# peterdavidfagan/mujoco_robot_environments

Measured on AMD Instinct MI355X. Metric: env steps/sec (whole node), RearrangementEnv batch=4096 at 1/2/4/8 MI355X, higher is better.
Workload: dtype f32

## Files before the change

### mujoco_robot_environments_amd/csrc/mre_api.cpp

```cpp
#include <hip/hip_runtime.h>

#include <cmath>
#include <cstdio>
#include <cstdlib>
#include <cstring>
#include <string>
#include <algorithm>
#include <vector>

#include "mre_env.h"
#include "mre_launch.h"
#include "mre_model.h"

using namespace mre;

static thread_local std::string g_err;
int mre::fail(int code, const std::string& msg) {
  g_err = msg;
  return code;
}

extern "C" const char* mre_last_error(void) { return g_err.c_str(); }

static int create_buffers(mre_env* e, int num_envs, int device_id) {
// ... 20 lines not shown
  HIPCHK(hipStreamCreateWithFlags(&e->stream2, hipStreamNonBlocking));
  HIPCHK(hipEventCreateWithFlags(&e->ev_fork, hipEventDisableTiming));
  HIPCHK(hipEventCreateWithFlags(&e->ev_join, hipEventDisableTiming));
  HIPCHK(hipMalloc(&e->d_large, N)); HIPCHK(hipMalloc(&e->mask_r, N));
  HIPCHK(hipMalloc(&e->sv_qpos, N * NQP * 4)); HIPCHK(hipMalloc(&e->sv_qvel, N * NVP * 4));
  HIPCHK(hipMalloc(&e->sv_qacc_ws, N * NVP * 4)); HIPCHK(hipMalloc(&e->sv_ctrl, N * NU * 4));
  HIPCHK(hipMalloc(&e->sv_status, N * 4));
  HIPCHK(hipMalloc(&e->sv_converged, N));
  HIPCHK(hipHostMalloc((void**)&e->h_launch_info, mre_env::RING * N * 16, hipHostMallocMapped | hipHostMallocCoherent));
  HIPCHK(hipHostGetDevicePointer((void**)&e->d_launch_info, e->h_launch_info, 0));
  memset(e->h_launch_info, 0xFF, mre_env::RING * N * 16);
  HIPCHK(hipHostMalloc((void**)&e->h_info_last, N * 16, hipHostMallocDefault));
  memset(e->h_info_last, 0xFF, N * 16);
  HIPCHK(hipHostMalloc((void**)&e->h_large_stage, mre_env::NSTAGE * N, hipHostMallocMapped | hipHostMallocCoherent));
  HIPCHK(hipHostGetDevicePointer((void**)&e->d_large_stage, e->h_large_stage, 0));
  memset(e->h_large_stage, 0, mre_env::NSTAGE * N);
  HIPCHK(hipMalloc(&e->d_pending, N));
  HIPCHK(hipMemsetAsync(e->d_pending, 0, N, e->stream));
  HIPCHK(hipMemsetAsync(e->d_large, 0, N, e->stream));
  e->h_large.assign(N, 0); e->h_rerun.assign(N, 0);
  { int rc = sched_create(e); if (rc) return rc; }
  if (const char* fb = getenv("MRE_NO_FALLBACK")) e->fallback = atoi(fb) == 0;
  if (const char* ng = getenv("MRE_NARROW_GENERIC")) e->base_flags = atoi(ng) != 0 ? F_CLIP_ALWAYS : 0u;
  if (const char* ng = getenv("MRE_NEWTON_GENERIC")) e->base_flags |= atoi(ng) != 0 ? F_NW_ALL_TILES : 0u;
  if (const char* fl = getenv("MRE_FORCE_LARGE")) {
    if (atoi(fl) != 0) {
      e->h_large.assign(N, 1); e->n_large = num_envs;
      HIPCHK(hipMemsetAsync(e->d_large, 1, N, e->stream));
    }
  }
  HIPCHK(hipMemsetAsync(e->status, 0, N * 4, e->stream)); HIPCHK(hipMemsetAsync(e->stats, 0, N * 16, e->stream));
  HIPCHK(hipMemsetAsync(e->grip_closed, 0, N, e->stream)); HIPCHK(hipMemsetAsync(e->osc_target, 0, N * 64, e->stream));
  HIPCHK(hipMemsetAsync(e->sites, 0, N * 64, e->stream));
  std::vector<int> np(N, NPROP);
  std::vector<float> ps(N * NPROP * 3, 0.0155f);
  HIPCHK(hipMemcpy(e->nprops, np.data(), N * 4, hipMemcpyHostToDevice));
  HIPCHK(hipMemcpy(e->prop_size, ps.data(), ps.size() * 4, hipMemcpyHostToDevice));
  e->osc = OscConfig{350.f, 20.f, 500.f, 100.f, 200.f, 30.f, {0.f, -0.785f, 0.f, -2.356f, 0.f, 1.571f, 0.785f},
                     5e-3f, 68e-3f, 0};
  HIPCHK(hipMalloc(&e->d_osc, sizeof(OscConfig)));
  HIPCHK(hipMemcpy(e->d_osc, &e->osc, sizeof(OscConfig), hipMemcpyHostToDevice));
  HIPCHK(hipStreamSynchronize(e->stream));
  int rc = mre_reset(e, nullptr);
  if (rc != MRE_OK) return rc;
  return mre_sync(e);
}
// ... 993 lines not shown
```

### mujoco_robot_environments_amd/csrc/mre_collide.h

```cpp
#pragma once
#include "mre_math.h"

namespace mre {

constexpr int COLL_BUF = 48;
MRE_DEV float* cand_xyz(float* buf, int k) { return buf + 24 + 3 * k; }
MRE_DEV float& cand_dist(float* buf, int k) { return buf[3 * k + 2]; }

struct FaceCand { float x[4], y[4], z[4], d[4]; };
constexpr unsigned FACE_IN_REGS = 16u;
constexpr unsigned FACE_BRANCH = 32u;

MRE_DEV float sel3(const float* v, int i) {
  const float w0 = i == 0 ? 1.f : 0.f, w1 = i == 1 ? 1.f : 0.f, w2 = i == 2 ? 1.f : 0.f;
  return w0 * v[0] + w1 * v[1] + w2 * v[2];
}
MRE_DEV void row3(float* o, const float (*m)[3], int i) {
  const float w0 = i == 0 ? 1.f : 0.f, w1 = i == 1 ? 1.f : 0.f, w2 = i == 2 ? 1.f : 0.f;
  o[0] = w0 * m[0][0] + w1 * m[1][0] + w2 * m[2][0];
  o[1] = w0 * m[0][1] + w1 * m[1][1] + w2 * m[2][1];
  o[2] = w0 * m[0][2] + w1 * m[1][2] + w2 * m[2][2];
}

MRE_DEV int clip_poly(float* p, float* q, int n, float sx, float sy) {
// ... 307 lines not shown
    for (int k = 0; k < 3; k++) x[k] += t * a[k];
  }
  if (wn > 1e-4f) {
    for (int k = 0; k < 3; k++) x[k] -= r * w[k] / wn;
  } else {
    float o[3];
    for (int k = 0; k < 3; k++) o[k] = fminf(fmaxf(x[k], -sb[k]), sb[k]) - x[k];
    const float oa = o[0] * a[0] + o[1] * a[1] + o[2] * a[2];
    for (int k = 0; k < 3; k++) o[k] -= oa * a[k];
    const float on = sqrtf(o[0] * o[0] + o[1] * o[1] + o[2] * o[2]);
    const float sc = on > r ? r / on : 1.f;
    for (int k = 0; k < 3; k++) x[k] += sc * o[k];
  }
  for (int k = 0; k < 3; k++) x[k] -= 0.5f * best * bd[k];
  float* c0 = cand_xyz(buf, 0);
  for (int k = 0; k < 3; k++) {
    c0[k] = pb[k] + Rb[3 * k] * x[0] + Rb[3 * k + 1] * x[1] + Rb[3 * k + 2] * x[2];
    normal[k] = Rb[3 * k] * bd[0] + Rb[3 * k + 1] * bd[1] + Rb[3 * k + 2] * bd[2];
  }
  cand_dist(buf, 0) = best;
  return 1;
}

MRE_DEV void make_frame(float* f) {
  float y[3] = {0.f, 0.f, 0.f};
  if (f[1] < 0.5f && f[1] > -0.5f) y[1] = 1.f; else y[2] = 1.f;
  const float t = v3dot(f, y);
  v3addscl(y, f, -t);
  v3normalize(y);
  v3copy(f + 3, y);
  v3cross(f + 6, f, f + 3);
}

}
```

### mujoco_robot_environments_amd/csrc/mre_dev.h

```cpp
#pragma once
#include <stdint.h>

namespace mre {

constexpr int NB = 20;
constexpr int NRB = 16;
constexpr int GRIP_BODY0 = 8;
constexpr int NV = 39;
constexpr int NRV = 15;
constexpr int NQ = 43;
constexpr int NQP = 44;
constexpr int TRACE_W = 88;
constexpr int TRACE_QVEL = 48;
constexpr int NVP = 40;
constexpr int NU = 8;
constexpr int QFINE = 32;
constexpr int QFINE_ROW = 96;
constexpr int QFINE_CUBE_Q = 32;
constexpr int QFINE_CUBE_V = 60;
static_assert(QFINE_CUBE_Q + 7 * 4 == QFINE_CUBE_V && QFINE_CUBE_V + 6 * 4 <= QFINE_ROW, "qfine row layout");
constexpr int NPROP = 4;
constexpr int NG = 20;
constexpr int PROP_GEOM0 = 12;
constexpr int NPAIR = 128;
// ... 132 lines not shown
  PairRec pair_rec[NPAIR];
  float act_ctrlrange[NU][2];
  float home_qpos[7];
  float park_pos[NPROP][3];
  BodyRec body_rec[NB];
  DofRec dof_rec[NV];
  MEntryRec m_rec[NMR];
  RowRec row_rec[NROWREC];
  EqRec eq_rec[NEQ];
  SiteRec site_rec[NSITE];
  OptRec opt_rec;
};

struct OscConfig {
  float kp_pos, kd_pos, kp_ori, kd_ori, kp_null, kd_null;
  float null_q[7];
  float pos_thresh, ori_thresh;
  int pinv_always;
};

enum StepFlags : unsigned { F_NO_CONSTRAINTS = 1u, F_FREEZE_ROBOT = 2u, F_CONV_CONTINUE = 4u, F_CONV_OPEN = 8u,
                            F_OSC_EVAL = 16u, F_DETECT = 32u, F_SETTLE_EXIT = 64u, F_DETECT_ACTIVE = 128u,
                            F_CLIP_ALWAYS = 256u, F_NW_ALL_TILES = 512u };
enum CtrlMode : int { CTRL_HELD = 0, CTRL_SEQ = 1, CTRL_OSC = 2 };

struct StepArgs {
  const DevModel* M;
  int N;
  float* qpos;
  float* qvel;
  float* qacc_ws;
  float* qfine;
  float* ctrl;
  const float* ctrl_seq;
  int seq_stride;
  const int* nprops;
  const float* prop_size;
  int nsteps, control_steps, mode;
  unsigned flags;
  const OscConfig* osc;
  int osc_stride;
  const float* osc_target;
  const uint8_t* grip_closed;
  uint8_t* converged;
  float* sites;
  uint32_t* status;
// ... 114 lines not shown
```

### mujoco_robot_environments_amd/csrc/mre_kernels.hip

```cpp
#include <hip/hip_runtime.h>

#include "mre_dev.h"
#include "mre_math.h"
#include "mre_collide.h"

namespace mre {
using ModelP = MRE_MODEL_PTR(DevModel);
#if defined(MRE_PHASE_STAMPS) && MRE_PHASE_STAMPS >= 4
__shared__ unsigned long long dbg_acc[4];
#endif

struct OscSm {
  float J[6][7], M[7][7], MiJt[7][6], Li[6][6], Lam[6][6], V[6][6], Jbar[7][6];
  float ep[3], eo[3], F[6], LF[6], tn[7], Jbt[6], xd[6], w[6];
};

struct alignas(8) Blk {
  uint16_t row0;
  uint8_t type, nrows;
  uint8_t rslot;
  uint8_t pa, pb;
  uint8_t primary : 4;
  uint8_t bslot : 4;
};
// ... 1374 lines not shown
  for (int step = step_lo; step < step_hi; ++step) {
    MRE_STAMP(7);
    position_stage(M, s, l);
    MRE_STAMP(12);
    MRE_STAMP(13);
    gripper_local(M, s, l);
    if ((a.flags & F_NO_CONSTRAINTS) == 0) connect_rows_local(M, s, l);
    MRE_STAMP(14);
    crb_mass_matrix(M, s, l);
    MRE_SYNC();
#ifndef MRE_NEWTON
    factor_robot_regs(s.qM, s.qLD, s.qLDinv);
#endif
    MRE_STAMP(15);
    MRE_STAMP(0);

    velocity_stage(M, s, l);
    MRE_SYNC();
    finger_bias(M, s, l);
    MRE_STAMP(1);
    const bool constrained = (a.flags & F_NO_CONSTRAINTS) == 0;
    if (constrained) {

      collide(M, s, l, false, (a.flags & F_CLIP_ALWAYS) != 0);
      MRE_STAMP(2);
      assemble_constraints(M, s, l);
#ifdef MRE_NEWTON
      nw_build_lists(s, l, a.flags);
#else
      solve_robot_rows(s, l);
      assemble_blocks(M, s, l);
#endif
      MRE_STAMP(3);
      hw_ncon = max(hw_ncon, s.ncon); hw_nefc = max(hw_nefc, s.nefc);
      hw_nrrow = max(hw_nrrow, s.nrrow); hw_npp = max(hw_npp, s.npp);
    }

    if (a.mode == CTRL_SEQ && (step % a.control_steps) == 0) {
      const int tick = step / a.control_steps;
      if (l < NU) s.ctrl[l] = a.ctrl_seq[((size_t)tick * a.seq_stride + env) * NU + l];
      MRE_SYNC();
    }
    if (a.mode == CTRL_OSC && (step % a.control_steps) == 0) {
      if (step > 0 && osc_converged(M, s, oscp, s.osc_tgt)) arm_converged = true;
      osc_compute(M, s, osc, oscp, s.osc_tgt, l);
      if (l == 0) s.ctrl[NU - 1] = grip_cmd;
      MRE_SYNC();
// ... 69 lines not shown
    }
    if (settled) break;
  }
  MRE_STAMP(7);
  if (a.settle_steps != nullptr && l == 0) a.settle_steps[env] = settled ? steps_done : -steps_done;
  const bool hand_over = QUEUE && !Q_LARGE && s.overflow != 0;
  if (a.nstep != nullptr && l == 0 && !hand_over) {
    if (QUEUE) __hip_atomic_fetch_add(a.nstep + env, steps_done, __ATOMIC_RELAXED, __HIP_MEMORY_SCOPE_AGENT);
    else a.nstep[env] += steps_done;
  }
  if (a.nsteps == 0 && (a.flags & F_OSC_EVAL) != 0 && a.mode == CTRL_OSC) {
    position_stage(M, s, l);
    gripper_local(M, s, l);
    crb_mass_matrix(M, s, l);
    MRE_SYNC();
    velocity_stage(M, s, l);
    MRE_SYNC();
    osc_compute(M, s, osc, oscp, s.osc_tgt, l);
    if (l == 0) s.ctrl[NU - 1] = grip_cmd;
    MRE_SYNC();
  }
  if (a.nsteps == 0 && (a.flags & F_DETECT) != 0 && a.contacts != nullptr) {
    position_stage(M, s, l);
    collide(M, s, l, (a.flags & F_DETECT_ACTIVE) == 0, (a.flags & F_CLIP_ALWAYS) != 0);
    float* o = a.contacts + (size_t)env * (1 + 3 * CONTACT_EXPORT);
    const int n = s.ncon < CONTACT_EXPORT ? s.ncon : CONTACT_EXPORT;
    if (l == 0) o[0] = s.overflow ? -(float)s.ncon : (float)s.ncon;
    if (l < n) {
      const int pr = s.con_pair[l];
      o[1 + 3 * l] = (float)M->pair_g1[pr]; o[2 + 3 * l] = (float)M->pair_g2[pr]; o[3 + 3 * l] = s.con_dist[l];
      if (a.contacts_full != nullptr) {
        float* f = a.contacts_full + ((size_t)env * CONTACT_EXPORT + l) * 12;
        for (int k = 0; k < 3; k++) f[k] = s.con_pos[l][k];
        for (int k = 0; k < 9; k++) f[3 + k] = s.con_frame[l][k];
      }
    }
    MRE_SYNC();
    if (l == 0) s.overflow = 0;
  }
  const bool q_last = !QUEUE || (qtick + 1 == a.q_nticks && !hand_over);
  if (q_last && (a.mode == CTRL_OSC || a.sites != nullptr || a.geoms != nullptr)) kinematics_only(M, s, l);
  if (a.mode == CTRL_OSC && a.nsteps > 0 && !hand_over) {
    if (q_last && osc_converged(M, s, oscp, s.osc_tgt)) arm_converged = true;
    if (l == 0) {
      if (a.converged != nullptr) a.converged[env] = arm_converged ? 1 : 0;
      if (q_last && !arm_converged && a.status != nullptr && (a.flags & F_CONV_OPEN) == 0) {
        if (QUEUE) __hip_atomic_fetch_or(a.status + env, 1u, __ATOMIC_RELAXED, __HIP_MEMORY_SCOPE_AGENT);
// ... 485 lines not shown
```

### mujoco_robot_environments_amd/csrc/mre_solver.h

```cpp
#pragma once

namespace mre {

constexpr int HDR_NONE = 0xFF;
constexpr int BLK_NONE = 0x7F;
constexpr int SCHED_NONE = 0xFF;
constexpr int TAB_OFF = MAXBLK * 5;
constexpr int TAB_ZEROS = 48;
static_assert(TAB_BYTES == 8 * (TAB_OFF + 1) + 4 * TAB_ZEROS, "operand table size");

#ifndef MRE_NEWTON
MRE_DEV void build_schedule(ModelP M, Sm& s);
#endif
MRE_DEV constexpr int cube_pair_bit(int p, int q) {
  const int a = p < q ? p : q, b = p < q ? q : p;
  return a == 0 ? b - 1 : (a == 1 ? b + 1 : 5);
}

MRE_DEV float prop_invM(const Sm& s, int p, int k) {
  return 1.0f / ((k < 3) ? s.prop_mass[p] : s.prop_inertia[p][k - 3]);
}

MRE_DEV void geom_pose(ModelP M, const Sm& s, int g, float* p, float* R, float* size,
                       float* rbound) {
// ... 6 lines not shown
  const int pid = M->geom_propid[g];
  if (pid >= 0) {
    v3copy(size, s.prop_size[pid]);
    *rbound = v3norm(size);
  } else {
    v3copy(size, M->geom_size[g]);
    *rbound = M->geom_rbound[g];
  }
}

MRE_DEV void geom_center(ModelP M, const Sm& s, int g, float* p, float* rbound) {
  const int b = M->geom_body[g];
  float tmp[3];
  m3mulv(tmp, s.xmat[b], M->geom_pos[g]);
  v3add(p, s.xpos[b], tmp);
  const int pid = M->geom_propid[g];
  *rbound = pid >= 0 ? v3norm(s.prop_size[pid]) : M->geom_rbound[g];
}

MRE_PHASE_FN int collide_broad(ModelP M, Sm& s, int l, bool detect) {
  static_assert(offsetof(Sm, hdr) + sizeof(((Sm*)0)->hdr) - offsetof(Sm, JpA) >= sizeof(float) * 64 * COLL_BUF,
                "clip buffers do not fit");
  static_assert(NPAIR <= 256 && sizeof(((Sm*)0)->iscr) >= NPAIR, "survivor list: one byte per pair");
  MRE_DBG_T0();
  uint8_t* list = reinterpret_cast<uint8_t*>(s.iscr);
  const unsigned long long lt = (1ull << l) - 1ull;
  int nsurv = 0;
  for (int pass = 0; pass < NPAIR / 64; pass++) {
    const int pr = l + 64 * pass;
    const auto* R = &M->pair_rec[pr];
    const int g1 = R->g1, b1 = R->b1, b2 = R->b2, pid1 = R->pid1, pid2 = R->pid2, type1 = R->type1;
    const float lp1[3] = {R->pos1[0], R->pos1[1], R->pos1[2]}, lp2[3] = {R->pos2[0], R->pos2[1], R->pos2[2]};
    const float mrb1 = R->rb1, mrb2 = R->rb2, margin = R->margin, gap = R->gap;
    const float lq1[4] = {R->quat1[0], R->quat1[1], R->quat1[2], R->quat1[3]};
    bool live = false;
    if (g1 >= 0 && (pid1 < 0 || pid1 < s.nprops) && (pid2 < 0 || pid2 < s.nprops)) {
      const float inc = detect ? margin : margin - gap;
      float p1[3], p2[3], df[3], tmp[3];
      m3mulv(tmp, s.xmat[b1], lp1); v3add(p1, s.xpos[b1], tmp);
      m3mulv(tmp, s.xmat[b2], lp2); v3add(p2, s.xpos[b2], tmp);
      const float rb1 = pid1 >= 0 ? v3norm(s.prop_size[pid1]) : mrb1, rb2 = pid2 >= 0 ? v3norm(s.prop_size[pid2]) : mrb2;
      v3sub(df, p2, p1);
      if (type1 == 0) {
        float q[4], R1[9];
        qmul(q, s.xquat[b1], lq1);
        q2mat(R1, q);
        const float nn[3] = {R1[2], R1[5], R1[8]};
        live = v3dot(df, nn) - rb2 <= inc;
      } else {
        const float r = rb1 + rb2 + inc;
        live = v3dot(df, df) <= r * r;
      }
    }
    const unsigned long long m = __ballot(live);
    if (live) list[nsurv + __popcll(m & lt)] = (uint8_t)pr;
    nsurv += __popcll(m);
  }
  if (l == 0) s.ncon = 0;
  MRE_SYNC();
  MRE_DBG_STAMP(6, 0);
  return nsurv;
}
MRE_PHASE_FN int collide_narrow(ModelP M, Sm& s, int l, bool detect, bool clip_always, int c0, int nsurv, int base) {
  MRE_DBG_T0();
  float* buf = &s.JpA[0][0] + l * COLL_BUF;
  const uint8_t* list = reinterpret_cast<const uint8_t*>(s.iscr);
  const unsigned long long lt = (1ull << l) - 1ull;
  {
    const int pr = (c0 + l < nsurv) ? list[c0 + l] : -1;
    float normal[3] = {0.f, 0.f, 1.f};
    int n = 0;
    FaceCand rc;
    unsigned rm = 0u;
    if (pr >= 0) {
      const auto* R = &M->pair_rec[pr];
      const int b1 = R->b1, b2 = R->b2, pid1 = R->pid1, pid2 = R->pid2, type1 = R->type1;
      const float lp1[3] = {R->pos1[0], R->pos1[1], R->pos1[2]}, lp2[3] = {R->pos2[0], R->pos2[1], R->pos2[2]};
      const float lq1[4] = {R->quat1[0], R->quat1[1], R->quat1[2], R->quat1[3]};
      const float lq2[4] = {R->quat2[0], R->quat2[1], R->quat2[2], R->quat2[3]};
      const float ms1[3] = {R->size1[0], R->size1[1], R->size1[2]}, ms2[3] = {R->size2[0], R->size2[1], R->size2[2]};
      const float margin = R->margin, gap = R->gap;
      float p1[3], R1[9], s1[3], p2[3], R2[9], s2[3], tmp[3], q[4];
      m3mulv(tmp, s.xmat[b1], lp1); v3add(p1, s.xpos[b1], tmp);
      qmul(q, s.xquat[b1], lq1); q2mat(R1, q);
      m3mulv(tmp, s.xmat[b2], lp2); v3add(p2, s.xpos[b2], tmp);
      qmul(q, s.xquat[b2], lq2); q2mat(R2, q);
      if (pid1 >= 0) v3copy(s1, s.prop_size[pid1]); else v3copy(s1, ms1);
      if (pid2 >= 0) v3copy(s2, s.prop_size[pid2]); else v3copy(s2, ms2);
      const float inc = detect ? margin : margin - gap;
      MRE_DBG_STAMP(6, 1);
      if ((R->single >> 8) == 2) n = cyl_box(p1, R1, s1, p2, R2, s2[0], s2[2], inc, normal, buf);
      else if (type1 == 0) n = plane_box(p1, R1, p2, R2, s2, inc, normal, buf);
      else n = box_box(p1, R1, s1, p2, R2, s2, inc, normal, buf, clip_always, rc, rm);
      MRE_DBG_STAMP(6, 2);
      int m = 0;
      if (rm & FACE_IN_REGS) {
#pragma unroll
        for (int v = 0; v < 4; v++) {
          if (((rm >> v) & 1u) != 0u && rc.d[v] < inc) m++;
          else rm &= ~(1u << v);
        }
      } else {
        for (int c = 0; c < n; c++)
          if (cand_dist(buf, c) < inc) {
            if (m != c) {
              for (int k = 0; k < 3; k++) cand_xyz(buf, m)[k] = cand_xyz(buf, c)[k];
              cand_dist(buf, m) = cand_dist(buf, c);
            }
            m++;
          }
      }
      n = m;
    }
#if defined(MRE_PHASE_STAMPS) && MRE_PHASE_STAMPS == 8
    {
      const bool tbl = pr >= 0 && (M->pair_rec[pr].g1 == 1);
      const unsigned long long fb = __ballot((rm & FACE_BRANCH) != 0u), fr = __ballot((rm & FACE_IN_REGS) != 0u), tb = __ballot(tbl);
      if (l == 0) {
        dbg_acc[0] += (unsigned long long)__popcll(fb) << 4; dbg_acc[1] += (unsigned long long)__popcll(fr) << 4;
        dbg_acc[2] += (unsigned long long)__popcll(fb & tb) << 4; dbg_acc[3] += (unsigned long long)__popcll(fr & tb) << 4;
      }
    }
#endif
    const bool single = pr >= 0 && n > 1 && (M->pair_rec[pr].single & 0xFF) != 0;
    const int ncand = n;
    if (single) n = 1;
    int off = base, tot = base;
    for (int bit = 0; bit < 4; bit++) {
      const unsigned long long m = __ballot((n >> bit) & 1);
      off += __popcll(m & lt) << bit;
      tot += __popcll(m) << bit;
    }
    if (l == 0) {
      s.ncon = tot < NCON_MAX ? tot : NCON_MAX;
      if (tot > NCON_MAX) s.overflow = 1;
    }
    if (single) {
      const float incw = M->pair_rec[pr].margin - M->pair_rec[pr].gap;
      if (rm & FACE_IN_REGS) {
        float wsum = 0.f, px = 0.f, py = 0.f, pz = 0.f, dmin = 0.f, bx = 0.f, by = 0.f, bz = 0.f;
        bool first = true;
#pragma unroll
        for (int v = 0; v < 4; v++)
          if (((rm >> v) & 1u) != 0u) {
            const float dc = rc.d[v];
            if (first || dc < dmin) { dmin = dc; bx = rc.x[v]; by = rc.y[v]; bz = rc.z[v]; }
            first = false;
            const float w = incw - dc;
            if (w > 0.f) { wsum += w; px += w * rc.x[v]; py += w * rc.y[v]; pz += w * rc.z[v]; }
          }
        if (wsum > 0.f) { const float iw = 1.0f / wsum; px *= iw; py *= iw; pz *= iw; }
        else { px = bx; py = by; pz = bz; }
        rc.x[0] = px; rc.y[0] = py; rc.z[0] = pz; rc.d[0] = dmin;
        rm = FACE_IN_REGS | 1u;
      } else {
        float wsum = 0.f, px = 0.f, py = 0.f, pz = 0.f, dmin = cand_dist(buf, 0);
        int best = 0;
        for (int c = 0; c < ncand; c++) {
          const float dc = cand_dist(buf, c);
          if (dc < dmin) { dmin = dc; best = c; }
          const float w = incw - dc;
          if (w > 0.f) { wsum += w; px += w * cand_xyz(buf, c)[0]; py += w * cand_xyz(buf, c)[1]; pz += w * cand_xyz(buf, c)[2]; }
        }
        if (wsum > 0.f) { const float iw = 1.0f / wsum; px *= iw; py *= iw; pz *= iw; }
        else { px = cand_xyz(buf, best)[0]; py = cand_xyz(buf, best)[1]; pz = cand_xyz(buf, best)[2]; }
        cand_xyz(buf, 0)[0] = px; cand_xyz(buf, 0)[1] = py; cand_xyz(buf, 0)[2] = pz;
        cand_dist(buf, 0) = dmin;
      }
    }
    if (n > 0) {
      float f[9];
      v3copy(f, normal);
      make_frame(f);
      if (rm & FACE_IN_REGS) {
        int id = off;
#pragma unroll
        for (int v = 0; v < 4; v++)
          if (((rm >> v) & 1u) != 0u && id < NCON_MAX) {
            s.con_pos[id][0] = rc.x[v]; s.con_pos[id][1] = rc.y[v]; s.con_pos[id][2] = rc.z[v];
            for (int k = 0; k < 9; k++) s.con_frame[id][k] = f[k];
            s.con_dist[id] = rc.d[v];
            s.con_pair[id] = (uint8_t)pr;
            id++;
          }
      } else {
        for (int c = 0; c < n; c++) {
          const int id = off + c;
          if (id >= NCON_MAX) break;
          const float cx0 = cand_xyz(buf, c)[0], cx1 = cand_xyz(buf, c)[1], cx2 = cand_xyz(buf, c)[2];
          s.con_pos[id][0] = cx0; s.con_pos[id][1] = cx1; s.con_pos[id][2] = cx2;
          for (int k = 0; k < 9; k++) s.con_frame[id][k] = f[k];
          s.con_dist[id] = cand_dist(buf, c);
          s.con_pair[id] = (uint8_t)pr;
        }
      }
    }
    MRE_SYNC();
    MRE_DBG_STAMP(6, 3);
    return tot;
  }
}
MRE_DEV void collide(ModelP M, Sm& s, int l, bool detect, bool clip_always) {
  const int nsurv = collide_broad(M, s, l, detect);
  int base = 0;
  for (int c0 = 0; c0 < nsurv; c0 += 64) {
    base = collide_narrow(M, s, l, detect, clip_always, c0, nsurv, base);
    if (base > NCON_MAX) break;
  }
}

MRE_DEV float impedance(const float* solimp, float pos, float margin) {
  const float dmin = clampf(solimp[0], 0.0001f, 0.9999f), dmax = clampf(solimp[1], 0.0001f, 0.9999f);
  const float width = fmaxf(solimp[2], kMinVal), mid = clampf(solimp[3], 0.0001f, 0.9999f);
  const float power = fmaxf(solimp[4], 1.0f);
  if (dmin == dmax) return 0.5f * (dmin + dmax);
  const float x = fabsf((pos - margin) / width);
  if (x >= 1.0f) return dmax;
  if (x <= 0.0f) return dmin;
  float y;
  if (power == 1.0f) y = x;
  else if (power == 2.0f) {
    y = (x <= mid) ? x * x / mid : 1.0f - (1.0f - x) * (1.0f - x) / (1.0f - mid);
  }
  else if (x <= mid) y = powf(x, power) / powf(mid, power - 1.0f);
  else y = 1.0f - powf(1.0f - x, power) / powf(1.0f - mid, power - 1.0f);
  return dmin + y * (dmax - dmin);
}

MRE_DEV void jac_robot(ModelP M, Sm& s, int rs, int b, const float* p, const float* ax, float sg) {
// ... 82 lines not shown
  }
  MRE_SYNC();
}

#endif

constexpr int GRIP0 = GRIP_BODY0;

MRE_PHASE_FN void assemble_constraints(ModelP M, Sm& s, int l) {
  int lim = 0, lim_side = 0;
  const auto* BR = &M->body_rec[l < NRB ? l : 0];
  const int jnt_limited = BR->jnt_limited;
  const float jnt_range[2] = {BR->jnt_range[0], BR->jnt_range[1]};
  if (l >= 1 && l < NRB && jnt_limited) {
    const double q = robot_q(s, l - 1);
    if (q - (double)jnt_range[0] < 0.0) { lim = 1; lim_side = -1; }
    else if ((double)jnt_range[1] - q < 0.0) { lim = 1; lim_side = 1; }
  }
  keep_live(jnt_range[0]); keep_live(jnt_range[1]);
  const unsigned long long limm = __ballot(lim != 0);
  const int lim_idx = __popcll(limm & ((1ull << l) - 1ull));
  if (l == 0) s.nl = __popcll(limm);
  if (lim) s.lim_info[lim_idx] = l | ((lim_side > 0 ? 1 : 0) << 8);
  if (l < s.ncon) {
    const int pr = s.con_pair[l];
    s.con_b1[l] = (uint8_t)M->pair_rec[pr].b1;
    s.con_b2[l] = (uint8_t)M->pair_rec[pr].b2;
  }
  MRE_SYNC();
#ifndef MRE_NEWTON
  {
    static_assert(sizeof(s.sched) % 4 == 0, "schedule cleared by words");
    unsigned* w = reinterpret_cast<unsigned*>(&s.sched[0][0]);
    for (int e = l; e < (int)(sizeof(s.sched) / 4); e += 64) w[e] = 0x01010101u * (unsigned)SCHED_NONE;
  }
#endif
  {
    const int base = 7 + s.nl, ncon0 = s.ncon;
    const bool on = l < ncon0;
    const int cb1 = on ? s.con_b1[l] : 0, cb2 = on ? s.con_b2[l] : 0;
    const bool rob_any = on && ((cb1 < NRB && cb1 > 0) || (cb2 < NRB && cb2 > 0));
    const bool fing = on && ((cb1 >= GRIP_BODY0 && cb1 < NRB) || (cb2 >= GRIP_BODY0 && cb2 < NRB));
    const unsigned long long fingm = __ballot(fing);
    const bool two_props = on && cb1 >= NRB && cb2 >= NRB;
    const unsigned long long lt = (1ull << l) - 1ull;
    const unsigned long long rmask = __ballot(rob_any), tmask = __ballot(two_props);
    const int my_r = base + 3 * __popcll(rmask & lt), my_b = __popcll(tmask & lt);
    const bool fail = on && (base + 3 * (l + 1) > NEFC_MAX || (rob_any && my_r + 3 > NRROW_MAX) ||
                             (two_props && my_b >= NPP_MAX));
    const unsigned long long fmask = __ballot(fail);
    const int kept = fmask != 0ull ? (int)__builtin_ctzll(fmask) : ncon0;
// ... 715 lines not shown
```

Baseline: 25.85 million.

## Split box-box narrowphase across four lanes per pair for small survivor counts

Adds a quad-lane narrowphase path in which four lanes cooperate on one box-box pair: the face SAT runs per lane, the edge axes are split by row, and face vertices are evaluated one per lane, with results combined through cross-lane reads. When the number of surviving pairs in the last chunk is small (up to a configurable count, default 16), those pairs use the quad path, so that the wavefront's otherwise idle lanes share the per-pair work. Contact body indices are now written during narrowphase rather than looked up again in assemble_constraints. The cost is extra cross-lane shuffles and more code and register pressure in the collision stage.

```diff
diff --git a/mujoco_robot_environments_amd/csrc/mre_api.cpp b/mujoco_robot_environments_amd/csrc/mre_api.cpp
--- a/mujoco_robot_environments_amd/csrc/mre_api.cpp
+++ b/mujoco_robot_environments_amd/csrc/mre_api.cpp
@@ -66,6 +66,7 @@
   { int rc = sched_create(e); if (rc) return rc; }
   if (const char* fb = getenv("MRE_NO_FALLBACK")) e->fallback = atoi(fb) == 0;
   if (const char* ng = getenv("MRE_NARROW_GENERIC")) e->base_flags = atoi(ng) != 0 ? F_CLIP_ALWAYS : 0u;
+  if (const char* nq = getenv("MRE_NARROW_QUAD_MAX")) e->base_flags |= (unsigned)(16 - std::clamp(atoi(nq), 0, 16)) << F_QUAD_SHIFT;
   if (const char* ng = getenv("MRE_NEWTON_GENERIC")) e->base_flags |= atoi(ng) != 0 ? F_NW_ALL_TILES : 0u;
   if (const char* fl = getenv("MRE_FORCE_LARGE")) {
     if (atoi(fl) != 0) {
diff --git a/mujoco_robot_environments_amd/csrc/mre_collide.h b/mujoco_robot_environments_amd/csrc/mre_collide.h
--- a/mujoco_robot_environments_amd/csrc/mre_collide.h
+++ b/mujoco_robot_environments_amd/csrc/mre_collide.h
@@ -353,6 +353,230 @@
   return 1;
 }
 
+
+MRE_DEV float pick3(float v0, float v1, float v2, int i) {
+  const unsigned m0 = i == 0 ? ~0u : 0u, m1 = i == 1 ? ~0u : 0u, m2 = i == 2 ? ~0u : 0u;
+  const unsigned u = (__builtin_bit_cast(unsigned, v0) & m0) | (__builtin_bit_cast(unsigned, v1) & m1) |
+                     (__builtin_bit_cast(unsigned, v2) & m2);
+  return __builtin_bit_cast(float, u);
+}
+
+struct BoxSat {
+  float A[3][3], B[3][3], dv[3], aC[3][3], tA[3], tB[3];
+  float best_face;
+  int face_code;
+};
+MRE_DEV void box_sat_faces(const float* p1, const float* R1, const float* s1, const float* p2, const float* R2,
+                           const float* s2, BoxSat& S) {
+  float Cm[3][3];
+#pragma unroll
+  for (int i = 0; i < 3; i++)
+#pragma unroll
+    for (int k = 0; k < 3; k++) { S.A[i][k] = R1[3 * k + i]; S.B[i][k] = R2[3 * k + i]; }
+  v3sub(S.dv, p2, p1);
+#pragma unroll
+  for (int i = 0; i < 3; i++)
+#pragma unroll
+    for (int j = 0; j < 3; j++) { Cm[i][j] = v3dot(S.A[i], S.B[j]); S.aC[i][j] = fabsf(Cm[i][j]); }
+#pragma unroll
+  for (int i = 0; i < 3; i++) { S.tA[i] = v3dot(S.dv, S.A[i]); S.tB[i] = v3dot(S.dv, S.B[i]); }
+  float best_face = -1e30f;
+  int face_code = -1;
+#pragma unroll
+  for (int i = 0; i < 3; i++) {
+    const float sep = fabsf(S.tA[i]) - (s1[i] + s2[0] * S.aC[i][0] + s2[1] * S.aC[i][1] + s2[2] * S.aC[i][2]);
+    if (sep > best_face) { best_face = sep; face_code = i; }
+  }
+#pragma unroll
+  for (int j = 0; j < 3; j++) {
+    const float sep = fabsf(S.tB[j]) - (s2[j] + s1[0] * S.aC[0][j] + s1[1] * S.aC[1][j] + s1[2] * S.aC[2][j]);
+    if (sep > best_face) { best_face = sep; face_code = 3 + j; }
+  }
+  S.best_face = best_face;
+  S.face_code = face_code;
+}
+
+struct EdgeBest {
+  float best;
+  int ej;
+  float en[3];
+  bool separated;
+};
+MRE_DEV void edge_axes_row(const BoxSat& S, const float* s1, const float* s2, float margin, int i, EdgeBest& E) {
+  const int i1 = i >= 2 ? i - 2 : i + 1, i2 = i >= 1 ? i - 1 : i + 2;
+  float Ai[3], aCi[3], aCi1[3], aCi2[3];
+#pragma unroll
+  for (int k = 0; k < 3; k++) {
+    Ai[k] = pick3(S.A[0][k], S.A[1][k], S.A[2][k], i);
+    aCi[k] = pick3(S.aC[0][k], S.aC[1][k], S.aC[2][k], i);
+    aCi1[k] = pick3(S.aC[0][k], S.aC[1][k], S.aC[2][k], i1);
+    aCi2[k] = pick3(S.aC[0][k], S.aC[1][k], S.aC[2][k], i2);
+  }
+  const float s1i1 = pick3(s1[0], s1[1], s1[2], i1), s1i2 = pick3(s1[0], s1[1], s1[2], i2);
+  E.best = -1e30f;
+  E.ej = -1;
+  E.en[0] = E.en[1] = E.en[2] = 0.f;
+  E.separated = false;
+#pragma unroll
+  for (int j = 0; j < 3; j++) {
+    float L[3];
+    v3cross(L, Ai, S.B[j]);
+    const float len = v3norm(L);
+    if (len >= 1e-6f) {
+      const int j1 = (j + 1) % 3, j2 = (j + 2) % 3;
+      const float rA = s1i1 * aCi2[j] + s1i2 * aCi1[j];
+      const float rB = s2[j1] * aCi[j2] + s2[j2] * aCi[j1];
+      const float t = v3dot(S.dv, L);
+      const float sep = (fabsf(t) - rA - rB) / len;
+      if (sep > margin) E.separated = true;
+      if (sep > E.best) {
+        E.best = sep; E.ej = j;
+        const float sg = (t >= 0 ? 1.0f : -1.0f) / len;
+        E.en[0] = L[0] * sg; E.en[1] = L[1] * sg; E.en[2] = L[2] * sg;
+      }
+    }
+  }
+}
+MRE_DEV void edge_combine(float& best_edge, int& ei, int& ej, float* en, float row_best, int row_ej, const float* row_en, int i) {
+  if (row_best > best_edge) { best_edge = row_best; ei = i; ej = row_ej; en[0] = row_en[0]; en[1] = row_en[1]; en[2] = row_en[2]; }
+}
+MRE_DEV bool box_use_edge(float best_edge, float best_face, int ei) {
+  return (ei >= 0) && (best_edge - best_face > 0.05f * fabsf(best_face) + 1e-7f);
+}
+
+MRE_DEV int box_edge_contact(const BoxSat& S, const float* p1, const float* s1, const float* p2, const float* s2,
+                             int ei, int ej, const float* en, float margin, float* normal, float* c, float& dist) {
+  float c1[3], c2[3];
+  v3copy(c1, p1);
+  v3copy(c2, p2);
+#pragma unroll
+  for (int k = 0; k < 3; k++) {
+    if (k != ei) v3addscl(c1, S.A[k], (v3dot(en, S.A[k]) >= 0 ? 1.0f : -1.0f) * s1[k]);
+    if (k != ej) v3addscl(c2, S.B[k], (v3dot(en, S.B[k]) >= 0 ? -1.0f : 1.0f) * s2[k]);
+  }
+  float Ae[3], Be[3], w[3];
+  row3(Ae, S.A, ei);
+  row3(Be, S.B, ej);
+  v3sub(w, c1, c2);
+  const float uv = v3dot(Ae, Be), uw = v3dot(Ae, w), vw = v3dot(Be, w);
+  const float den = 1.0f - uv * uv;
+  float a = 0.f, bb = 0.f;
+  if (den > 1e-12f) { a = (uv * vw - uw) / den; bb = (vw - uv * uw) / den; }
+  float q1[3], q2[3], df[3];
+  v3copy(q1, c1); v3addscl(q1, Ae, a);
+  v3copy(q2, c2); v3addscl(q2, Be, bb);
+  v3copy(normal, en);
+  v3sub(df, q2, q1);
+  const float d = v3dot(df, en);
+  c[0] = 0.5f * (q1[0] + q2[0]); c[1] = 0.5f * (q1[1] + q2[1]); c[2] = 0.5f * (q1[2] + q2[2]);
+  dist = d;
+  return d <= margin ? 1 : 0;
+}
+
+struct FaceRef {
+  float nr[3], Aru[3], Arv[3], Aiu[3], Aiv[3], ci[3], cr[3];
+  float siu, siv, sru, srv;
+};
+MRE_DEV void box_face_setup(const BoxSat& S, const float* p1, const float* s1, const float* p2, const float* s2,
+                            float* normal, FaceRef& F) {
+  const bool ref1 = S.face_code < 3;
+  const int a = ref1 ? S.face_code : S.face_code - 3;
+  float pr[3], pi[3];
+#pragma unroll
+  for (int k = 0; k < 3; k++) { pr[k] = ref1 ? p1[k] : p2[k]; pi[k] = ref1 ? p2[k] : p1[k]; }
+  float Ar[3][3], Ai[3][3], srv3[3], siv3[3];
+#pragma unroll
+  for (int i = 0; i < 3; i++) {
+#pragma unroll
+    for (int k = 0; k < 3; k++) { Ar[i][k] = ref1 ? S.A[i][k] : S.B[i][k]; Ai[i][k] = ref1 ? S.B[i][k] : S.A[i][k]; }
+    srv3[i] = ref1 ? s1[i] : s2[i];
+    siv3[i] = ref1 ? s2[i] : s1[i];
+  }
+  float Ara[3];
+  row3(Ara, Ar, a);
+  {
+    const float ta = ref1 ? sel3(S.tA, a) : sel3(S.tB, a);
+    const float sg = ref1 ? (ta >= 0 ? 1.0f : -1.0f) : (ta >= 0 ? -1.0f : 1.0f);
+    for (int k = 0; k < 3; k++) { F.nr[k] = Ara[k] * sg; normal[k] = ref1 ? F.nr[k] : -F.nr[k]; }
+  }
+  int kk = 0;
+  float bestd = -1.f;
+#pragma unroll
+  for (int k = 0; k < 3; k++) {
+    const float dd = fabsf(v3dot(F.nr, Ai[k]));
+    if (dd > bestd) { bestd = dd; kk = k; }
+  }
+  const int ku = (kk + 1) % 3, kv = (kk + 2) % 3, au = (a + 1) % 3, av = (a + 2) % 3;
+  float Aik[3];
+  row3(Aik, Ai, kk); row3(F.Aiu, Ai, ku); row3(F.Aiv, Ai, kv);
+  row3(F.Aru, Ar, au); row3(F.Arv, Ar, av);
+  const float sik = sel3(siv3, kk);
+  F.siu = sel3(siv3, ku); F.siv = sel3(siv3, kv);
+  const float sra = sel3(srv3, a);
+  F.sru = sel3(srv3, au); F.srv = sel3(srv3, av);
+  const float isg = v3dot(F.nr, Aik) >= 0 ? -1.0f : 1.0f;
+  v3copy(F.ci, pi);
+  v3addscl(F.ci, Aik, isg * sik);
+  v3copy(F.cr, pr);
+  v3addscl(F.cr, F.nr, sra);
+}
+MRE_DEV void box_face_vertex(const FaceRef& F, int v, float& x, float& y, float& d) {
+  const float su = (v == 0 || v == 3) ? 1.0f : -1.0f;
+  const float sv = (v < 2) ? 1.0f : -1.0f;
+  float w[3];
+  v3copy(w, F.ci);
+  v3addscl(w, F.Aiu, su * F.siu);
+  v3addscl(w, F.Aiv, sv * F.siv);
+  v3sub(w, w, F.cr);
+  x = v3dot(w, F.Aru);
+  y = v3dot(w, F.Arv);
+  d = v3dot(w, F.nr);
+}
+MRE_DEV bool box_face_vertex_inside(const FaceRef& F, float x, float y) {
+  return clip_keeps(1.0f, x, F.sru) && clip_keeps(-1.0f, x, F.sru) && clip_keeps(1.0f, y, F.srv) && clip_keeps(-1.0f, y, F.srv);
+}
+MRE_DEV void box_face_candidate(const FaceRef& F, float x, float y, float dep, float* c) {
+  c[0] = F.cr[0] + x * F.Aru[0] + y * F.Arv[0] + 0.5f * dep * F.nr[0];
+  c[1] = F.cr[1] + x * F.Aru[1] + y * F.Arv[1] + 0.5f * dep * F.nr[1];
+  c[2] = F.cr[2] + x * F.Aru[2] + y * F.Arv[2] + 0.5f * dep * F.nr[2];
+}
+MRE_DEV int box_face_clip(const FaceRef& F, const float* vx, const float* vy, const float* vd, float margin, float* buf) {
+  float* poly = buf;
+#pragma unroll
+  for (int v = 0; v < 4; v++) { poly[3 * v] = vx[v]; poly[3 * v + 1] = vy[v]; poly[3 * v + 2] = vd[v]; }
+  const int n = clip_poly(poly, buf + 24, 4, F.sru, F.srv);
+  int nc = 0;
+  for (int v = 0; v < n; v++) {
+    const float x = poly[3 * v], y = poly[3 * v + 1], dep = poly[3 * v + 2];
+    if (dep > margin) continue;
+    float c[3];
+    box_face_candidate(F, x, y, dep, c);
+    float* cx = cand_xyz(buf, nc);
+    cx[0] = c[0]; cx[1] = c[1]; cx[2] = c[2];
+    cand_dist(buf, nc) = dep;
+    nc++;
+  }
+  return nc;
+}
+
+MRE_DEV void face_single(FaceCand& rc, unsigned& rm, float incw) {
+  float wsum = 0.f, px = 0.f, py = 0.f, pz = 0.f, dmin = 0.f, bx = 0.f, by = 0.f, bz = 0.f;
+  bool first = true;
+#pragma unroll
+  for (int v = 0; v < 4; v++)
+    if (((rm >> v) & 1u) != 0u) {
+      const float dc = rc.d[v];
+      if (first || dc < dmin) { dmin = dc; bx = rc.x[v]; by = rc.y[v]; bz = rc.z[v]; }
+      first = false;
+      const float w = incw - dc;
+      if (w > 0.f) { wsum += w; px += w * rc.x[v]; py += w * rc.y[v]; pz += w * rc.z[v]; }
+    }
+  if (wsum > 0.f) { const float iw = 1.0f / wsum; px *= iw; py *= iw; pz *= iw; }
+  else { px = bx; py = by; pz = bz; }
+  rc.x[0] = px; rc.y[0] = py; rc.z[0] = pz; rc.d[0] = dmin;
+  rm = FACE_IN_REGS | 1u;
+}
+
 MRE_DEV void make_frame(float* f) {
   float y[3] = {0.f, 0.f, 0.f};
   if (f[1] < 0.5f && f[1] > -0.5f) y[1] = 1.f; else y[2] = 1.f;
diff --git a/mujoco_robot_environments_amd/csrc/mre_dev.h b/mujoco_robot_environments_amd/csrc/mre_dev.h
--- a/mujoco_robot_environments_amd/csrc/mre_dev.h
+++ b/mujoco_robot_environments_amd/csrc/mre_dev.h
@@ -178,6 +178,7 @@
 enum StepFlags : unsigned { F_NO_CONSTRAINTS = 1u, F_FREEZE_ROBOT = 2u, F_CONV_CONTINUE = 4u, F_CONV_OPEN = 8u,
                             F_OSC_EVAL = 16u, F_DETECT = 32u, F_SETTLE_EXIT = 64u, F_DETECT_ACTIVE = 128u,
                             F_CLIP_ALWAYS = 256u, F_NW_ALL_TILES = 512u };
+constexpr unsigned F_QUAD_SHIFT = 16u, F_QUAD_BITS = 31u;
 enum CtrlMode : int { CTRL_HELD = 0, CTRL_SEQ = 1, CTRL_OSC = 2 };
 
 struct StepArgs {
diff --git a/mujoco_robot_environments_amd/csrc/mre_kernels.hip b/mujoco_robot_environments_amd/csrc/mre_kernels.hip
--- a/mujoco_robot_environments_amd/csrc/mre_kernels.hip
+++ b/mujoco_robot_environments_amd/csrc/mre_kernels.hip
@@ -1420,7 +1420,7 @@
     const bool constrained = (a.flags & F_NO_CONSTRAINTS) == 0;
     if (constrained) {
 
-      collide(M, s, l, false, (a.flags & F_CLIP_ALWAYS) != 0);
+      collide(M, s, l, false, a.flags);
       MRE_STAMP(2);
       assemble_constraints(M, s, l);
 #ifdef MRE_NEWTON
@@ -1536,7 +1536,7 @@
   }
   if (a.nsteps == 0 && (a.flags & F_DETECT) != 0 && a.contacts != nullptr) {
     position_stage(M, s, l);
-    collide(M, s, l, (a.flags & F_DETECT_ACTIVE) == 0, (a.flags & F_CLIP_ALWAYS) != 0);
+    collide(M, s, l, (a.flags & F_DETECT_ACTIVE) == 0, a.flags);
     float* o = a.contacts + (size_t)env * (1 + 3 * CONTACT_EXPORT);
     const int n = s.ncon < CONTACT_EXPORT ? s.ncon : CONTACT_EXPORT;
     if (l == 0) o[0] = s.overflow ? -(float)s.ncon : (float)s.ncon;
diff --git a/mujoco_robot_environments_amd/csrc/mre_solver.h b/mujoco_robot_environments_amd/csrc/mre_solver.h
--- a/mujoco_robot_environments_amd/csrc/mre_solver.h
+++ b/mujoco_robot_environments_amd/csrc/mre_solver.h
@@ -52,6 +52,8 @@
   static_assert(offsetof(Sm, hdr) + sizeof(((Sm*)0)->hdr) - offsetof(Sm, JpA) >= sizeof(float) * 64 * COLL_BUF,
                 "clip buffers do not fit");
   static_assert(NPAIR <= 256 && sizeof(((Sm*)0)->iscr) >= NPAIR, "survivor list: one byte per pair");
+  static_assert(offsetof(Sm, con_b1) + sizeof(((Sm*)0)->con_b1) <= offsetof(Sm, JpA) && offsetof(Sm, con_b2) + sizeof(((Sm*)0)->con_b2) <= offsetof(Sm, JpA),
+                "con_b1 / con_b2 must not lie in the clip buffers");
   MRE_DBG_T0();
   uint8_t* list = reinterpret_cast<uint8_t*>(s.iscr);
   const unsigned long long lt = (1ull << l) - 1ull;
@@ -91,7 +93,45 @@
   MRE_DBG_STAMP(6, 0);
   return nsurv;
 }
-MRE_PHASE_FN int collide_narrow(ModelP M, Sm& s, int l, bool detect, bool clip_always, int c0, int nsurv, int base) {
+MRE_DEV int cand_filter(float* buf, int n, float inc) {
+  int m = 0;
+  for (int c = 0; c < n; c++)
+    if (cand_dist(buf, c) < inc) {
+      if (m != c) {
+        for (int k = 0; k < 3; k++) cand_xyz(buf, m)[k] = cand_xyz(buf, c)[k];
+        cand_dist(buf, m) = cand_dist(buf, c);
+      }
+      m++;
+    }
+  return m;
+}
+MRE_DEV void cand_single(float* buf, int ncand, float incw) {
+  float wsum = 0.f, px = 0.f, py = 0.f, pz = 0.f, dmin = cand_dist(buf, 0);
+  int best = 0;
+  for (int c = 0; c < ncand; c++) {
+    const float dc = cand_dist(buf, c);
+    if (dc < dmin) { dmin = dc; best = c; }
+    const float w = incw - dc;
+    if (w > 0.f) { wsum += w; px += w * cand_xyz(buf, c)[0]; py += w * cand_xyz(buf, c)[1]; pz += w * cand_xyz(buf, c)[2]; }
+  }
+  if (wsum > 0.f) { const float iw = 1.0f / wsum; px *= iw; py *= iw; pz *= iw; }
+  else { px = cand_xyz(buf, best)[0]; py = cand_xyz(buf, best)[1]; pz = cand_xyz(buf, best)[2]; }
+  cand_xyz(buf, 0)[0] = px; cand_xyz(buf, 0)[1] = py; cand_xyz(buf, 0)[2] = pz;
+  cand_dist(buf, 0) = dmin;
+}
+MRE_DEV void cand_store(Sm& s, float* buf, int n, int off, const float* f, int pr, int bodies) {
+  for (int c = 0; c < n; c++) {
+    const int id = off + c;
+    if (id >= NCON_MAX) break;
+    const float cx0 = cand_xyz(buf, c)[0], cx1 = cand_xyz(buf, c)[1], cx2 = cand_xyz(buf, c)[2];
+    s.con_pos[id][0] = cx0; s.con_pos[id][1] = cx1; s.con_pos[id][2] = cx2;
+    for (int k = 0; k < 9; k++) s.con_frame[id][k] = f[k];
+    s.con_dist[id] = cand_dist(buf, c);
+    s.con_pair[id] = (uint8_t)pr;
+    s.con_b1[id] = (uint8_t)bodies; s.con_b2[id] = (uint8_t)(bodies >> 8);
+  }
+}
+MRE_DEV int collide_narrow_lanes(ModelP M, Sm& s, int l, bool detect, bool clip_always, int c0, int nsurv, int base) {
   MRE_DBG_T0();
   float* buf = &s.JpA[0][0] + l * COLL_BUF;
   const uint8_t* list = reinterpret_cast<const uint8_t*>(s.iscr);
@@ -102,14 +142,19 @@
     int n = 0;
     FaceCand rc;
     unsigned rm = 0u;
+    int single_w = 0, bodies = 0;
+    float incw = 0.f;
     if (pr >= 0) {
       const auto* R = &M->pair_rec[pr];
       const int b1 = R->b1, b2 = R->b2, pid1 = R->pid1, pid2 = R->pid2, type1 = R->type1;
+      bodies = b1 | (b2 << 8);
+      single_w = R->single;
       const float lp1[3] = {R->pos1[0], R->pos1[1], R->pos1[2]}, lp2[3] = {R->pos2[0], R->pos2[1], R->pos2[2]};
       const float lq1[4] = {R->quat1[0], R->quat1[1], R->quat1[2], R->quat1[3]};
       const float lq2[4] = {R->quat2[0], R->quat2[1], R->quat2[2], R->quat2[3]};
       const float ms1[3] = {R->size1[0], R->size1[1], R->size1[2]}, ms2[3] = {R->size2[0], R->size2[1], R->size2[2]};
       const float margin = R->margin, gap = R->gap;
+      incw = margin - gap;
       float p1[3], R1[9], s1[3], p2[3], R2[9], s2[3], tmp[3], q[4];
       m3mulv(tmp, s.xmat[b1], lp1); v3add(p1, s.xpos[b1], tmp);
       qmul(q, s.xquat[b1], lq1); q2mat(R1, q);
@@ -119,29 +164,23 @@
       if (pid2 >= 0) v3copy(s2, s.prop_size[pid2]); else v3copy(s2, ms2);
       const float inc = detect ? margin : margin - gap;
       MRE_DBG_STAMP(6, 1);
-      if ((R->single >> 8) == 2) n = cyl_box(p1, R1, s1, p2, R2, s2[0], s2[2], inc, normal, buf);
+      if ((single_w >> 8) == 2) n = cyl_box(p1, R1, s1, p2, R2, s2[0], s2[2], inc, normal, buf);
       else if (type1 == 0) n = plane_box(p1, R1, p2, R2, s2, inc, normal, buf);
       else n = box_box(p1, R1, s1, p2, R2, s2, inc, normal, buf, clip_always, rc, rm);
       MRE_DBG_STAMP(6, 2);
-      int m = 0;
       if (rm & FACE_IN_REGS) {
+        int m = 0;
 #pragma unroll
         for (int v = 0; v < 4; v++) {
           if (((rm >> v) & 1u) != 0u && rc.d[v] < inc) m++;
           else rm &= ~(1u << v);
         }
+        n = m;
       } else {
-        for (int c = 0; c < n; c++)
-          if (cand_dist(buf, c) < inc) {
-            if (m != c) {
-              for (int k = 0; k < 3; k++) cand_xyz(buf, m)[k] = cand_xyz(buf, c)[k];
-              cand_dist(buf, m) = cand_dist(buf, c);
-            }
-            m++;
-          }
-      }
-      n = m;
-    }
+        n = cand_filter(buf, n, inc);
+      }
+    }
+    keep_live(single_w); keep_live(incw);
 #if defined(MRE_PHASE_STAMPS) && MRE_PHASE_STAMPS == 8
     {
       const bool tbl = pr >= 0 && (M->pair_rec[pr].g1 == 1);
@@ -152,7 +191,7 @@
       }
     }
 #endif
-    const bool single = pr >= 0 && n > 1 && (M->pair_rec[pr].single & 0xFF) != 0;
+    const bool single = pr >= 0 && n > 1 && (single_w & 0xFF) != 0;
     const int ncand = n;
     if (single) n = 1;
     int off = base, tot = base;
@@ -166,36 +205,10 @@
       if (tot > NCON_MAX) s.overflow = 1;
     }
     if (single) {
-      const float incw = M->pair_rec[pr].margin - M->pair_rec[pr].gap;
       if (rm & FACE_IN_REGS) {
-        float wsum = 0.f, px = 0.f, py = 0.f, pz = 0.f, dmin = 0.f, bx = 0.f, by = 0.f, bz = 0.f;
-        bool first = true;
-#pragma unroll
-        for (int v = 0; v < 4; v++)
-          if (((rm >> v) & 1u) != 0u) {
-            const float dc = rc.d[v];
-            if (first || dc < dmin) { dmin = dc; bx = rc.x[v]; by = rc.y[v]; bz = rc.z[v]; }
-            first = false;
-            const float w = incw - dc;
-            if (w > 0.f) { wsum += w; px += w * rc.x[v]; py += w * rc.y[v]; pz += w * rc.z[v]; }
-          }
-        if (wsum > 0.f) { const float iw = 1.0f / wsum; px *= iw; py *= iw; pz *= iw; }
-        else { px = bx; py = by; pz = bz; }
-        rc.x[0] = px; rc.y[0] = py; rc.z[0] = pz; rc.d[0] = dmin;
-        rm = FACE_IN_REGS | 1u;
+        face_single(rc, rm, incw);
       } else {
-        float wsum = 0.f, px = 0.f, py = 0.f, pz = 0.f, dmin = cand_dist(buf, 0);
-        int best = 0;
-        for (int c = 0; c < ncand; c++) {
-          const float dc = cand_dist(buf, c);
-          if (dc < dmin) { dmin = dc; best = c; }
-          const float w = incw - dc;
-          if (w > 0.f) { wsum += w; px += w * cand_xyz(buf, c)[0]; py += w * cand_xyz(buf, c)[1]; pz += w * cand_xyz(buf, c)[2]; }
-        }
-        if (wsum > 0.f) { const float iw = 1.0f / wsum; px *= iw; py *= iw; pz *= iw; }
-        else { px = cand_xyz(buf, best)[0]; py = cand_xyz(buf, best)[1]; pz = cand_xyz(buf, best)[2]; }
-        cand_xyz(buf, 0)[0] = px; cand_xyz(buf, 0)[1] = py; cand_xyz(buf, 0)[2] = pz;
-        cand_dist(buf, 0) = dmin;
+        cand_single(buf, ncand, incw);
       }
     }
     if (n > 0) {
@@ -211,18 +224,11 @@
             for (int k = 0; k < 9; k++) s.con_frame[id][k] = f[k];
             s.con_dist[id] = rc.d[v];
             s.con_pair[id] = (uint8_t)pr;
+            s.con_b1[id] = (uint8_t)bodies; s.con_b2[id] = (uint8_t)(bodies >> 8);
             id++;
           }
       } else {
-        for (int c = 0; c < n; c++) {
-          const int id = off + c;
-          if (id >= NCON_MAX) break;
-          const float cx0 = cand_xyz(buf, c)[0], cx1 = cand_xyz(buf, c)[1], cx2 = cand_xyz(buf, c)[2];
-          s.con_pos[id][0] = cx0; s.con_pos[id][1] = cx1; s.con_pos[id][2] = cx2;
-          for (int k = 0; k < 9; k++) s.con_frame[id][k] = f[k];
-          s.con_dist[id] = cand_dist(buf, c);
-          s.con_pair[id] = (uint8_t)pr;
-        }
+        cand_store(s, buf, n, off, f, pr, bodies);
       }
     }
     MRE_SYNC();
@@ -230,11 +236,198 @@
     return tot;
   }
 }
-MRE_DEV void collide(ModelP M, Sm& s, int l, bool detect, bool clip_always) {
+template <int SRC>
+MRE_DEV float quad_get(float v) { return dpp_row<0x55 * SRC>(v); }
+template <int SRC>
+MRE_DEV int quad_get(int v) { return __builtin_amdgcn_update_dpp(0, v, 0x55 * SRC, 0xF, 0xF, false); }
+MRE_DEV int quad_and(int v) {
+  v &= __builtin_amdgcn_update_dpp(0, v, 0xB1, 0xF, 0xF, false);
+  return v & __builtin_amdgcn_update_dpp(0, v, 0x4E, 0xF, 0xF, false);
+}
+MRE_DEV int collide_narrow_quad(ModelP M, Sm& s, int l, bool detect, int c0, int nsurv, int base) {
+  MRE_DBG_T0();
+  const int q = l & 3;
+  float* buf = &s.JpA[0][0] + (l & ~3) * COLL_BUF;
+  const uint8_t* list = reinterpret_cast<const uint8_t*>(s.iscr);
+  const unsigned long long lt = (1ull << l) - 1ull;
+  const int slot = c0 + (l >> 2);
+  const int pr = slot < nsurv ? list[slot] : -1;
+  float normal[3] = {0.f, 0.f, 1.f};
+  int n = 0;
+  bool reg = false;
+  float cx[3] = {0.f, 0.f, 0.f}, cd = 0.f;
+  int single_w = 0, bodies = 0;
+  float incw = 0.f;
+#if defined(MRE_PHASE_STAMPS)
+  bool dbg_face = false, dbg_clip = false;
+#endif
+  if (pr >= 0) {
+    const auto* R = &M->pair_rec[pr];
+    const int b1 = R->b1, b2 = R->b2, pid1 = R->pid1, pid2 = R->pid2, type1 = R->type1;
+    bodies = b1 | (b2 << 8);
+    single_w = R->single;
+    const float lp1[3] = {R->pos1[0], R->pos1[1], R->pos1[2]}, lp2[3] = {R->pos2[0], R->pos2[1], R->pos2[2]};
+    const float lq1[4] = {R->quat1[0], R->quat1[1], R->quat1[2], R->quat1[3]};
+    const float lq2[4] = {R->quat2[0], R->quat2[1], R->quat2[2], R->quat2[3]};
+    const float ms1[3] = {R->size1[0], R->size1[1], R->size1[2]}, ms2[3] = {R->size2[0], R->size2[1], R->size2[2]};
+    const float margin = R->margin, gap = R->gap;
+    incw = margin - gap;
+    float p1[3], R1[9], s1[3], p2[3], R2[9], s2[3], tmp[3], qq[4];
+    m3mulv(tmp, s.xmat[b1], lp1); v3add(p1, s.xpos[b1], tmp);
+    qmul(qq, s.xquat[b1], lq1); q2mat(R1, qq);
+    m3mulv(tmp, s.xmat[b2], lp2); v3add(p2, s.xpos[b2], tmp);
+    qmul(qq, s.xquat[b2], lq2); q2mat(R2, qq);
+    if (pid1 >= 0) v3copy(s1, s.prop_size[pid1]); else v3copy(s1, ms1);
+    if (pid2 >= 0) v3copy(s2, s.prop_size[pid2]); else v3copy(s2, ms2);
+    const float inc = detect ? margin : margin - gap;
+    MRE_DBG_STAMP(6, 1);
+    if ((single_w >> 8) == 2) {
+      if (q == 0) n = cyl_box(p1, R1, s1, p2, R2, s2[0], s2[2], inc, normal, buf);
+    } else if (type1 == 0) {
+      if (q == 0) n = plane_box(p1, R1, p2, R2, s2, inc, normal, buf);
+    } else {
+      BoxSat S;
+      box_sat_faces(p1, R1, s1, p2, R2, s2, S);
+      if (!(S.best_face > inc)) {
+        EdgeBest E;
+        edge_axes_row(S, s1, s2, inc, q, E);
+        float best_edge = -1e30f, en[3] = {0.f, 0.f, 0.f};
+        int ei = -1, ej = -1;
+        {
+          const float r0[3] = {quad_get<0>(E.en[0]), quad_get<0>(E.en[1]), quad_get<0>(E.en[2])};
+          const float r1[3] = {quad_get<1>(E.en[0]), quad_get<1>(E.en[1]), quad_get<1>(E.en[2])};
+          const float r2[3] = {quad_get<2>(E.en[0]), quad_get<2>(E.en[1]), quad_get<2>(E.en[2])};
+          edge_combine(best_edge, ei, ej, en, quad_get<0>(E.best), quad_get<0>(E.ej), r0, 0);
+          edge_combine(best_edge, ei, ej, en, quad_get<1>(E.best), quad_get<1>(E.ej), r1, 1);
+          edge_combine(best_edge, ei, ej, en, quad_get<2>(E.best), quad_get<2>(E.ej), r2, 2);
+        }
+        const int sep = E.separated ? 1 : 0;
+        const bool separated = (quad_get<0>(sep) | quad_get<1>(sep) | quad_get<2>(sep)) != 0;
+        if (!separated) {
+          if (box_use_edge(best_edge, S.best_face, ei)) {
+            const int k = box_edge_contact(S, p1, s1, p2, s2, ei, ej, en, inc, normal, cx, cd);
+            reg = true;
+            n = (q == 0 && k > 0 && cd < inc) ? 1 : 0;
+          } else {
+            FaceRef F;
+            box_face_setup(S, p1, s1, p2, s2, normal, F);
+            float vx, vy, vd;
+            box_face_vertex(F, q, vx, vy, vd);
+#if defined(MRE_PHASE_STAMPS)
+            dbg_face = true;
+#endif
+            if (quad_and(box_face_vertex_inside(F, vx, vy) ? 1 : 0) != 0) {
+              box_face_candidate(F, vx, vy, vd, cx);
+              cd = vd;
+              reg = true;
+              n = (!(vd > inc) && vd < inc) ? 1 : 0;
+            } else {
+              const float gx[4] = {quad_get<0>(vx), quad_get<1>(vx), quad_get<2>(vx), quad_get<3>(vx)};
+              const float gy[4] = {quad_get<0>(vy), quad_get<1>(vy), quad_get<2>(vy), quad_get<3>(vy)};
+              const float gd[4] = {quad_get<0>(vd), quad_get<1>(vd), quad_get<2>(vd), quad_get<3>(vd)};
+              if (q == 0) n = box_face_clip(F, gx, gy, gd, inc, buf);
+#if defined(MRE_PHASE_STAMPS)
+              dbg_clip = true;
+#endif
+            }
+          }
+        }
+      }
+    }
+    MRE_DBG_STAMP(6, 2);
+    if (!reg && n > 0) n = cand_filter(buf, n, inc);
+  }
+  keep_live(single_w); keep_live(incw);
+  const unsigned long long regs = __ballot(reg && n > 0);
+  const unsigned rmq = (unsigned)(regs >> (l & ~3)) & 0xFu;
+#if defined(MRE_PHASE_STAMPS) && MRE_PHASE_STAMPS == 8
+  {
+    const bool tbl = pr >= 0 && (M->pair_rec[pr].g1 == 1);
+    const unsigned long long fb = __ballot(dbg_face && q == 0), fr = __ballot(dbg_face && !dbg_clip && q == 0), tb = __ballot(tbl);
+    if (l == 0) {
+      dbg_acc[0] += (unsigned long long)__popcll(fb) << 4; dbg_acc[1] += (unsigned long long)__popcll(fr) << 4;
+      dbg_acc[2] += (unsigned long long)__popcll(fb & tb) << 4; dbg_acc[3] += (unsigned long long)__popcll(fr & tb) << 4;
+    }
+  }
+#endif
+#if defined(MRE_PHASE_STAMPS) && MRE_PHASE_STAMPS == 12
+  {
+    const unsigned long long cb = __ballot(dbg_clip && q == 0);
+    if (l == 0) dbg_acc[3] += (unsigned long long)__popcll(cb) << 4;
+  }
+#endif
+  const int npair = reg ? __popc(rmq) : n;
+  const bool single = pr >= 0 && npair > 1 && (single_w & 0xFF) != 0;
+  if (single) {
+    if (reg) {
+      FaceCand rc;
+      rc.x[0] = quad_get<0>(cx[0]); rc.x[1] = quad_get<1>(cx[0]); rc.x[2] = quad_get<2>(cx[0]); rc.x[3] = quad_get<3>(cx[0]);
+      rc.y[0] = quad_get<0>(cx[1]); rc.y[1] = quad_get<1>(cx[1]); rc.y[2] = quad_get<2>(cx[1]); rc.y[3] = quad_get<3>(cx[1]);
+      rc.z[0] = quad_get<0>(cx[2]); rc.z[1] = quad_get<1>(cx[2]); rc.z[2] = quad_get<2>(cx[2]); rc.z[3] = quad_get<3>(cx[2]);
+      rc.d[0] = quad_get<0>(cd); rc.d[1] = quad_get<1>(cd); rc.d[2] = quad_get<2>(cd); rc.d[3] = quad_get<3>(cd);
+      unsigned rm = FACE_IN_REGS | rmq;
+      face_single(rc, rm, incw);
+      cx[0] = rc.x[0]; cx[1] = rc.y[0]; cx[2] = rc.z[0]; cd = rc.d[0];
+      n = q == 0 ? 1 : 0;
+    } else {
+      cand_single(buf, n, incw);
+      n = 1;
+    }
+  }
+  int off = base, tot = base;
+  for (int bit = 0; bit < 4; bit++) {
+    const unsigned long long m = __ballot((n >> bit) & 1);
+    off += __popcll(m & lt) << bit;
+    tot += __popcll(m) << bit;
+  }
+  if (l == 0) {
+    s.ncon = tot < NCON_MAX ? tot : NCON_MAX;
+    if (tot > NCON_MAX) s.overflow = 1;
+  }
+  if (n > 0) {
+    float f[9];
+    v3copy(f, normal);
+    make_frame(f);
+    if (reg) {
+      if (off < NCON_MAX) {
+        s.con_pos[off][0] = cx[0]; s.con_pos[off][1] = cx[1]; s.con_pos[off][2] = cx[2];
+        for (int k = 0; k < 9; k++) s.con_frame[off][k] = f[k];
+        s.con_dist[off] = cd;
+        s.con_pair[off] = (uint8_t)pr;
+        s.con_b1[off] = (uint8_t)bodies; s.con_b2[off] = (uint8_t)(bodies >> 8);
+      }
+    } else {
+      cand_store(s, buf, n, off, f, pr, bodies);
+    }
+  }
+  MRE_SYNC();
+  MRE_DBG_STAMP(6, 3);
+  return tot;
+}
+constexpr int QUAD_PAIRS = 16;
+MRE_PHASE_FN int collide_narrow(ModelP M, Sm& s, int l, bool detect, int qmode, int c0, int nsurv, int base) {
+  qmode = __builtin_amdgcn_readfirstlane(qmode);
+  c0 = __builtin_amdgcn_readfirstlane(c0);
+  nsurv = __builtin_amdgcn_readfirstlane(nsurv);
+  const int rem = nsurv - c0;
+  int end = nsurv;
+  if (qmode >= 0 && rem <= 64) end = rem <= qmode ? c0 : (qmode < QUAD_PAIRS ? nsurv - qmode : nsurv);
+#if defined(MRE_PHASE_STAMPS) && MRE_PHASE_STAMPS == 12
+  if (l == 0) {
+    const unsigned long long np = (end > c0 ? 1ull : 0ull) + (end < nsurv ? 1ull : 0ull);
+    dbg_acc[0] += np << 4; if (end < nsurv) dbg_acc[1] += 16ull; if (rem > QUAD_PAIRS) dbg_acc[2] += 16ull;
+  }
+#endif
+  if (end > c0) base = collide_narrow_lanes(M, s, l, detect, qmode < 0, c0, end, base);
+  if (end < nsurv && __builtin_amdgcn_readfirstlane(base) <= NCON_MAX) base = collide_narrow_quad(M, s, l, detect, end, nsurv, base);
+  return base;
+}
+MRE_DEV void collide(ModelP M, Sm& s, int l, bool detect, unsigned flags) {
   const int nsurv = collide_broad(M, s, l, detect);
+  const int qmode = (flags & F_CLIP_ALWAYS) != 0 ? -1 : QUAD_PAIRS - (int)((flags >> F_QUAD_SHIFT) & F_QUAD_BITS);
   int base = 0;
   for (int c0 = 0; c0 < nsurv; c0 += 64) {
-    base = collide_narrow(M, s, l, detect, clip_always, c0, nsurv, base);
+    base = collide_narrow(M, s, l, detect, qmode, c0, nsurv, base);
     if (base > NCON_MAX) break;
   }
 }
@@ -363,11 +556,6 @@
   const int lim_idx = __popcll(limm & ((1ull << l) - 1ull));
   if (l == 0) s.nl = __popcll(limm);
   if (lim) s.lim_info[lim_idx] = l | ((lim_side > 0 ? 1 : 0) << 8);
-  if (l < s.ncon) {
-    const int pr = s.con_pair[l];
-    s.con_b1[l] = (uint8_t)M->pair_rec[pr].b1;
-    s.con_b2[l] = (uint8_t)M->pair_rec[pr].b2;
-  }
   MRE_SYNC();
 #ifndef MRE_NEWTON
   {
```

Result: no change. 25.91 million (median of 4 runs) (+0.2%).
